# DeepGraphLearning/RNNLogic

Hardware: NVIDIA B200
Metric: rule_grounded_train_queries_per_sec (higher is better)
Workload: dtype u32/f32

## Files before the change

### rnnlogic_b200/csrc/rl_kernels.cu

```cuda
#include "rl_device.cuh"
#include <stdlib.h>

static thread_local char g_err[512] = "";
static long long g_launches = 0;

int rl_fail(int code, const char *what, cudaError_t e)
{
    if (e != cudaSuccess) snprintf(g_err, sizeof(g_err), "%s: %s", what, cudaGetErrorString(e));
    else snprintf(g_err, sizeof(g_err), "%s", what);
    return code;
}
void rl_count_launch() { ++g_launches; }
static int fail(int code, const char *what, cudaError_t e = cudaSuccess) { return rl_fail(code, what, e); }

__global__ void k_prepare_slots(rl_graph g, int S, const int32_t *__restrict__ slot_head,
                                const int32_t *__restrict__ q_off, const int64_t *__restrict__ all_h,
                                const int64_t *__restrict__ all_t, const int64_t *__restrict__ etr, int remove_query_edges,
                                int32_t *lane_h, int32_t *lane_t, int32_t *lane_eh, int32_t *lane_et)
{
    int i = blockIdx.x * blockDim.x + threadIdx.x;
    if (i >= S * RL_LANES) return;
    int s = i >> 5, lane = i & 31;
    int qi = q_off[s] + lane;
    bool valid = qi < q_off[s + 1];
    int64_t hv = valid ? all_h[qi] : -1, tv = (valid && all_t) ? all_t[qi] : -1;
    if (hv < 0 || hv >= g.num_entities) hv = -1;
    if (tv < 0 || tv >= g.num_entities) tv = -1;
    lane_h[i] = (int32_t)hv;
    lane_t[i] = (int32_t)tv;
    int eh = -1, et = -1;
    const int rel = slot_head[s];
    if (valid && etr) {
        int64_t k = etr[qi];
        int64_t n = g.ord_ptr[rel + 1] - g.ord_ptr[rel];
        if (k >= 0 && k < n) {
            eh = g.ord_h[g.ord_ptr[rel] + k];
            et = g.ord_t[g.ord_ptr[rel] + k];
        }
    } else if (valid && remove_query_edges && hv >= 0 && tv >= 0) {
        const int row = rank_row(g, rel, (int)tv);
        if (row >= 0) {
            const long long grow = g.dst_ptr[rel] + row;
            for (long long k = g.row_start[grow]; k < g.row_start[grow + 1]; ++k)
                if (g.edge_src[k] == (int)hv) { eh = (int)hv; et = (int)tv; break; }
        }
    }
    lane_eh[i] = eh;
    lane_et[i] = et;
}

__device__ __forceinline__ int srank_row(const rl_graph &g, int rel, int e)
{
    const uint2 w = __ldg(reinterpret_cast<const uint2 *>(g.srank_tab) + (size_t)rel * g.rank_words + (e >> 5));
    const uint32_t bit = 1u << (e & 31);
    return (w.x & bit) ? (int)(w.y + __popc(w.x & (bit - 1))) : -1;
}

__device__ __forceinline__ void mark_out_edges(const rl_graph &g, int rho, int ent, uint32_t *cm)
{
    const int sr = srank_row(g, rho, ent);
    if (sr < 0) return;
    const int fb = g.fsrc_ptr[rho] + sr;
    const int k1 = g.frow_start[fb + 1];
    for (int k = g.frow_start[fb]; k < k1; ++k) {
        const int dr = __ldg(g.fedge_dstrow + k);
        atomicOr(cm + (dr >> 5), 1u << (dr & 31));
    }
}

template <bool ROOT>
__global__ void __launch_bounds__(WARPS_PER_BLOCK * 32)
k_symbolic(rl_graph g, rl_rules r, rl_slots s, int depth, rl_frontier fr, int dense_num, int dense_den, int force_dense)
{
    const int lane = threadIdx.x & 31, warp = threadIdx.x >> 5;
    const int slot = blockIdx.y;
    const int q = s.slot_head[slot];
    const int32_t *ip = r.lvl_sym_ptr + (size_t)q * (r.max_len + 1);
    const int item = ip[depth - 1] + blockIdx.x * WARPS_PER_BLOCK + warp;
    if (item >= ip[depth]) return;
    const int v = r.sym_node[item], w0 = r.sym_w0[item];
    const int4 ra = __ldg(reinterpret_cast<const int4 *>(r.node_rec) + 2 * (size_t)v);
    const int4 rb4 = __ldg(reinterpret_cast<const int4 *>(r.node_rec) + 2 * (size_t)v + 1);
    const int rho = ra.x;
    const int D = rb4.x;
    const int nw = (D + 31) >> 5;
    if (nw == 0) return;
    const int hc0 = r.lvl_ptr[(size_t)q * (r.max_len + 1)];
    uint32_t *mbase = fr.row_mask + (size_t)s.mask_off[slot];
    uint32_t *cm = mbase + (rb4.y - hc0);
    const int nzb = s.nz_off[slot] - r.head_node_ptr[q];
    bool dense = force_dense != 0;
    const uint32_t *pm = nullptr;
    int rho_p = -1, Dp = 0;
    if (!ROOT) {
        const int p = ra.y;
        const int cntp = fr.node_cnt[nzb + p];
        if (!dense && cntp == 0) return;
        rho_p = ra.z;
        Dp = g.dst_ptr[rho_p + 1] - g.dst_ptr[rho_p];
        if ((long long)cntp * dense_den > (long long)Dp * dense_num) dense = true;
        pm = mbase + (rb4.z - hc0);
    }
    if (dense) {
        if (w0 == 0)
            for (int w = lane; w < nw; w += 32)
                cm[w] = (w == nw - 1 && (D & 31)) ? ((1u << (D & 31)) - 1u) : 0xffffffffu;
        return;
    }
    if (ROOT) {
        const int h = s.lane_h[slot * RL_LANES + lane];
        if (h >= 0) mark_out_edges(g, rho, h, cm);
    } else {
        const int nwp = (Dp + 31) >> 5;
        const int pb = g.dst_ptr[rho_p];
        const int wi = w0 + lane;
        uint32_t word = wi < nwp ? pm[wi] : 0u;
        const int mine = __popc(word);
        int P = mine;
#pragma unroll
        for (int o = 1; o < 32; o <<= 1) {
            const int t = __shfl_up_sync(FULL, P, o);
            if (lane >= o) P += t;
        }
        const int T = __shfl_sync(FULL, P, 31);
        const int first = P - mine;
        for (int base = 0; base < T; base += 32) {
            const int k = min(base + lane, T - 1);
            int src_lane = 0;
#pragma unroll
            for (int step = 16; step > 0; step >>= 1)
                if (__shfl_sync(FULL, P, src_lane + step - 1) <= k) src_lane += step;
            const uint32_t wsel = __shfl_sync(FULL, word, src_lane);
            const int nth = k - __shfl_sync(FULL, first, src_lane);
            if (base + lane < T) {
                const int bit = __fns(wsel, 0, nth + 1);
                mark_out_edges(g, rho, __ldg(g.row_dst + pb + (w0 + src_lane) * 32 + bit), cm);
            }
        }
    }
}

#define EDGE_GROUP 8
#ifndef NUM_WARPS
#define NUM_WARPS 4
#endif
template <typename CT, bool ROOT, bool PRUNE>
__device__ __forceinline__ uint32_t numeric_rows(const rl_graph &g, const rl_rules &r, const rl_slots &s, const rl_frontier &fr,
                                                 int slot, int q, int hc0, const uint32_t *mbase, int v, int myrow,
                                                 int h, int lane_eh, int lane_et, bool &ovf)
{
    const int lane = threadIdx.x & 31;
    const int4 ra = __ldg(reinterpret_cast<const int4 *>(r.node_rec) + 2 * (size_t)v);
    const int4 rb4 = __ldg(reinterpret_cast<const int4 *>(r.node_rec) + 2 * (size_t)v + 1);
    const int rho = ra.x, prel = ra.z, nterm = rb4.w;
    const size_t abase = (size_t)s.arena_off[slot];
    CT *arena = reinterpret_cast<CT *>(fr.arena);
    const CT *__restrict__ X = nullptr;
    const uint32_t *__restrict__ pm = nullptr;
    if (!ROOT) {
        X = arena + (abase + (size_t)r.node_prow_off[v]) * RL_LANES;
        pm = mbase + (rb4.z - hc0);
    }
    CT *__restrict__ Y = arena + (abase + (size_t)r.node_row_off[v]) * RL_LANES;
    const bool active = myrow >= 0;
    const int grow = ra.w + max(myrow, 0);
    const int my_dst = active ? g.row_dst[grow] : -1;
    const bool masked = (rho == q);
    const int eh = masked ? lane_eh : -1;
    const int et = masked ? lane_et : -1;

    int cur = -1;
    unsigned long long acc = 0;
    uint32_t nzrows = 0;
    uint32_t my_lanes = 0;
    auto flush = [&](int j) {
        if (masked) {
            const int d = __shfl_sync(FULL, my_dst, j);
            if (eh >= 0 && et == d) {
                unsigned long long sub;
                if (ROOT) sub = (eh == h) ? 1ull : 0ull;
                else {
                    int pr = rank_row(g, prel, eh);
                    if (pr >= 0 && !((pm[pr >> 5] >> (pr & 31)) & 1u)) pr = -1;
                    sub = pr >= 0 ? (unsigned long long)X[(size_t)pr * RL_LANES + lane] : 0ull;
                }
                acc -= sub;
            }
        }
        if (sizeof(CT) == 4 && (acc >> 32)) ovf = true;
        const uint32_t nzl = __ballot_sync(FULL, acc != 0);
        if (!PRUNE || nzl) {
            Y[(size_t)__shfl_sync(FULL, myrow, j) * RL_LANES + lane] = (CT)acc;
            nzrows |= 1u << j;
            if (lane == j) my_lanes = nzl;
        }
        acc = 0;
    };

    constexpr bool SEARCH = ROOT && PRUNE;
    if (SEARCH) {
        int fs = 0, fe = 0;
        if (h >= 0) {
            const int sr = srank_row(g, rho, h);
            if (sr >= 0) {
                const int fb = g.fsrc_ptr[rho] + sr;
                fs = g.frow_start[fb];
                fe = g.frow_start[fb + 1];
            }
        }
        for (uint32_t act = __ballot_sync(FULL, active); act; act &= act - 1) {
            const int j = __ffs(act) - 1;
            const int rj = __shfl_sync(FULL, myrow, j);
            int lo = fs, hi = fe;
            while (lo < hi) {
                const int mid = (lo + hi) >> 1;
                if (__ldg(g.fedge_dstrow + mid) < rj) lo = mid + 1; else hi = mid;
            }
            int cnt = 0;
            while (lo + cnt < fe && __ldg(g.fedge_dstrow + lo + cnt) == rj) ++cnt;
            acc = (unsigned long long)cnt;
            flush(j);
        }
    } else {
    const int32_t *__restrict__ rs = ROOT ? g.row_start + grow : r.pair_ptr + (r.node_pair_off[v] + max(myrow, 0));
    const int my_rs = active ? rs[0] : 0;
    const int my_re = active ? rs[1] : 0;
    const int deg = my_re - my_rs;
    int P = deg;
#pragma unroll
    for (int o = 1; o < 32; o <<= 1) {
        const int t = __shfl_up_sync(FULL, P, o);
        if (lane >= o) P += t;
    }
    const int T = __shfl_sync(FULL, P, 31);
    const int my_first = P - deg;
    for (int base = 0; base < T; base += 32) {
        const int n = min(32, T - base);
        const int k = min(base + lane, T - 1);
        int row = 0;
#pragma unroll
        for (int step = 16; step > 0; step >>= 1)
            if (__shfl_sync(FULL, P, row + step - 1) <= k) row += step;
        const int e = __shfl_sync(FULL, my_rs, row) + (k - __shfl_sync(FULL, my_first, row));
        const int src = lane < n ? __ldg((ROOT ? g.edge_src : r.pair_ent) + e) : -1;
        int pr = -1;
        if (!ROOT && src >= 0 && ((pm[src >> 5] >> (src & 31)) & 1u)) pr = src;
        uint32_t todo = ROOT ? (n == 32 ? FULL : ((1u << n) - 1u)) : __ballot_sync(FULL, pr >= 0);
        while (todo) {
            CT vals[EDGE_GROUP];
            int rws[EDGE_GROUP];
#pragma unroll
            for (int u = 0; u < EDGE_GROUP; ++u) {
                const int kk = todo ? __ffs(todo) - 1 : -1;
                todo &= todo - 1;
                rws[u] = kk >= 0 ? __shfl_sync(FULL, row, kk) : -1;
                if (ROOT) {
                    const int sv = __shfl_sync(FULL, src, kk & 31);
                    vals[u] = (CT)((kk >= 0) && (sv == h));
                } else {
                    const int p = __shfl_sync(FULL, pr, kk & 31);
                    vals[u] = kk >= 0 ? X[(size_t)p * RL_LANES + lane] : (CT)0;
                }
            }
#pragma unroll
            for (int u = 0; u < EDGE_GROUP; ++u) {
                if (rws[u] >= 0) {
                    if (rws[u] != cur) {
                        if (cur >= 0) flush(cur);
                        cur = rws[u];
                    }
                    acc += (unsigned long long)vals[u];
                }
            }
        }
    }
    if (cur >= 0) flush(cur);
    }
    if (nterm > 0 && nzrows) {
        const bool mine = (nzrows >> lane) & 1u;
        if (fr.items) {
            const int term0 = __ldg(r.node_term_ptr + v);
            int base = 0;
            if (lane == 0) base = atomicAdd(fr.item_cnt + slot, __popc(nzrows));
            base = __shfl_sync(FULL, base, 0);
            if (mine) {
                const long long pos = fr.item_off[slot] + base + __popc(nzrows & ((1u << lane) - 1u));
                reinterpret_cast<int4 *>(fr.items)[pos] = make_int4((int)(r.node_row_off[v] + myrow), term0, my_dst, nterm);
                if (fr.item_mask) fr.item_mask[pos] = my_lanes;
                if (fr.bucket_cnt) atomicAdd(fr.bucket_cnt + (size_t)slot * RL_BUCKET_STRIDE(g.rank_words) + my_dst, 1);
                else if (fr.nzmask && my_lanes) atomicOr(fr.nzmask + (size_t)slot * g.num_entities + my_dst, my_lanes);
            }
        }
    }
    return nzrows;
}

template <typename CT, bool ROOT, bool PRUNE>
__global__ void __launch_bounds__(NUM_WARPS * 32, 48 / NUM_WARPS)
k_numeric(rl_graph g, rl_rules r, rl_slots s, int depth, rl_frontier fr, int cpw)
{
    const int lane = threadIdx.x & 31, warp = threadIdx.x >> 5;
    const int slot = blockIdx.y;
    const int q = s.slot_head[slot];
    const int32_t *lp = r.lvl_ptr + (size_t)q * (r.max_len + 1);
    const int c_end = lp[depth];
    const int c0 = lp[depth - 1] + (blockIdx.x * NUM_WARPS + warp) * cpw;
    if (c0 >= c_end) return;
    const int hc0 = lp[0];
    uint32_t *mbase = fr.row_mask + (size_t)s.mask_off[slot];
    const int nzb = s.nz_off[slot] - r.head_node_ptr[q];
    const int my_chunk = c0 + lane;
    const bool mine = lane < cpw && my_chunk < c_end;
    const uint32_t my_m = mine ? mbase[my_chunk - hc0] : 0u;
    uint32_t todo = __ballot_sync(FULL, my_m != 0u);
    if (todo == 0u) return;
    const int my_node = my_m ? r.chunk_node[my_chunk] : -1;
    const int my_row0 = my_m ? r.chunk_row0[my_chunk] : 0;
    const int h = s.lane_h[slot * RL_LANES + lane];
    const int leh = s.lane_eh[slot * RL_LANES + lane];
    const int let_ = s.lane_et[slot * RL_LANES + lane];
    bool ovf = false;
    int rows_done = 0;
    while (todo) {
        const int v = __shfl_sync(FULL, my_node, __ffs(todo) - 1);
        const uint32_t seg = __ballot_sync(FULL, my_m != 0u && my_node == v);
        todo &= ~seg;
        const int cnt = ((seg >> lane) & 1u) ? __popc(my_m) : 0;
        int P = cnt;
#pragma unroll
        for (int o = 1; o < 32; o <<= 1) {
            const int t = __shfl_up_sync(FULL, P, o);
            if (lane >= o) P += t;
        }
        const int V = __shfl_sync(FULL, P, 31);
        const int first = P - cnt;
        for (int g0 = 0; g0 < V; g0 += 32) {
            const bool have = g0 + lane < V;
            const int k = min(g0 + lane, V - 1);
            int sl = 0;
#pragma unroll
            for (int step = 16; step > 0; step >>= 1)
                if (__shfl_sync(FULL, P, sl + step - 1) <= k) sl += step;
            const uint32_t wsel = __shfl_sync(FULL, my_m, sl);
            const int nth = k - __shfl_sync(FULL, first, sl);
            const int r0 = __shfl_sync(FULL, my_row0, sl);
            const int bit = __fns(wsel, 0, nth + 1);
            const int myrow = have ? r0 + bit : -1;
            const uint32_t nz = numeric_rows<CT, ROOT, PRUNE>(g, r, s, fr, slot, q, hc0, mbase, v, myrow, h, leh, let_, ovf);
            if (have && !((nz >> lane) & 1u)) atomicAnd(mbase + (c0 + sl - hc0), ~(1u << bit));
            if (lane == 0 && nz) atomicAdd(fr.node_cnt + nzb + v, __popc(nz));
            rows_done += __popc(nz);
        }
    }
    if (lane == 0 && rows_done && depth < 8) atomicAdd(fr.overflow + 1 + depth, rows_done);
    if (__any_sync(FULL, ovf) && lane == 0) fr.overflow[0] = 1;
}

template <bool FILL>
__global__ void __launch_bounds__(128)
k_pair_table(rl_graph g, const int32_t *__restrict__ pair_prel, const int32_t *__restrict__ pair_rel,
             const int64_t *__restrict__ pair_base, const int32_t *__restrict__ ptr, int32_t *__restrict__ out)
{
    const int p = blockIdx.x;
    const int rp = pair_prel[p], rr = pair_rel[p];
    const long long base = pair_base[p];
    const int row0 = g.dst_ptr[rr], D = g.dst_ptr[rr + 1] - row0;
    for (int d = threadIdx.x; d < D; d += blockDim.x) {
        int n = 0;
        const int pos = FILL ? ptr[base + d] : 0;
        const int k1 = g.row_start[row0 + d + 1];
        for (int k = g.row_start[row0 + d]; k < k1; ++k) {
            const int pr = rank_row(g, rp, __ldg(g.edge_src + k));
            if (pr >= 0) {
                if (FILL) out[pos + n] = pr;
                ++n;
            }
        }
        if (!FILL) out[base + d] = n;
    }
    if (!FILL && threadIdx.x == 0) out[base + D] = 0;
}

__global__ void __launch_bounds__(WARPS_PER_BLOCK * 32)
k_propagate_dense(rl_graph g, int rel, int B, const int64_t *__restrict__ x, const int64_t *__restrict__ etr,
                  int64_t *__restrict__ out)
{
    const int lane = threadIdx.x & 31, warp = threadIdx.x >> 5;
    const int e = blockIdx.x * WARPS_PER_BLOCK + warp;
    if (e >= g.num_entities) return;
    const int row = rank_row(g, rel, e);
    const long long o0 = g.ord_ptr[rel], n_ord = g.ord_ptr[rel + 1] - o0;
    for (int b = lane; b < B; b += 32) {
        unsigned long long acc = 0;
        if (row >= 0) {
            const long long grow = g.dst_ptr[rel] + row;
            for (int k = g.row_start[grow]; k < g.row_start[grow + 1]; ++k)
                acc += (unsigned long long)x[(size_t)g.edge_src[k] * B + b];
            if (etr) {
                const long long k = etr[b];
                if (k >= 0 && k < n_ord && g.ord_t[o0 + k] == e) acc -= (unsigned long long)x[(size_t)g.ord_h[o0 + k] * B + b];
            }
        }
        out[(size_t)e * B + b] = (int64_t)acc;
    }
}

template <typename CT>
__global__ void k_node_dense(rl_graph g, rl_rules r, rl_slots s, int slot, int node, rl_frontier fr,
                             int64_t *__restrict__ out)
{
    __shared__ long long tile[32][33];
    const int lane = threadIdx.x & 31, w = threadIdx.x >> 5;
    const int N = g.num_entities;
    const int e = blockIdx.x * 32 + w;
    long long c = 0;
    if (e < N) {
        if (node < 0) c = (s.lane_h[slot * RL_LANES + lane] == e);
        else {
            const int q = s.slot_head[slot];
            const int hc0 = r.lvl_ptr[(size_t)q * (r.max_len + 1)];
            const uint32_t *mbase = fr.row_mask + (size_t)s.mask_off[slot];
            const int row = rank_row(g, r.node_rel[node], e);
            if (row >= 0 && row_valid(r.node_chunk0, mbase, hc0, node, row))
                c = (long long)reinterpret_cast<const CT *>(fr.arena)[((size_t)s.arena_off[slot] + r.node_row_off[node] + row) * RL_LANES + lane];
        }
    }
    tile[w][lane] = c;
    __syncthreads();
    const int eo = blockIdx.x * 32 + lane;
    if (eo < N) out[(size_t)w * N + eo] = tile[lane][w];
}

__global__ void __launch_bounds__(512)
k_items_scan(int W, rl_frontier fr)
{
    __shared__ int wsum[16];
    const int slot = blockIdx.x, tid = threadIdx.x, lane = tid & 31, warp = tid >> 5;
    int4 *cnt4 = reinterpret_cast<int4 *>(fr.bucket_cnt + (size_t)slot * RL_BUCKET_STRIDE(W));
    int4 *off4 = reinterpret_cast<int4 *>(fr.bucket_off + (size_t)slot * RL_BUCKET_STRIDE(W));
    int carry = 0;
    for (int w0 = 0; w0 < W; w0 += 512) {
        const int w = w0 + tid;
        int4 c[8];
        int sum = 0;
        if (w < W) {
#pragma unroll
            for (int k = 0; k < 8; ++k) {
                c[k] = cnt4[(size_t)w * 8 + k];
                sum += (c[k].x + c[k].y) + (c[k].z + c[k].w);
            }
        }
        int incl = sum;
#pragma unroll
        for (int o = 1; o < 32; o <<= 1) {
            const int v = __shfl_up_sync(FULL, incl, o);
            if (lane >= o) incl += v;
        }
        if (lane == 31) wsum[warp] = incl;
        __syncthreads();
        int wbase = 0, total = 0;
#pragma unroll
        for (int k = 0; k < 16; ++k) {
            const int v = wsum[k];
            if (k < warp) wbase += v;
            total += v;
        }
        int run = carry + wbase + incl - sum;
        if (w < W) {
#pragma unroll
            for (int k = 0; k < 8; ++k) {
                int4 o;
                o.x = run; run += c[k].x;
                o.y = run; run += c[k].y;
                o.z = run; run += c[k].z;
                o.w = run; run += c[k].w;
                off4[(size_t)w * 8 + k] = o;
                cnt4[(size_t)w * 8 + k] = make_int4(0, 0, 0, 0);
            }
        }
        carry += total;
        __syncthreads();
    }
    if (tid == 0) fr.bucket_off[(size_t)slot * RL_BUCKET_STRIDE(W) + (size_t)W * 32] = carry;
}

#define SCATTER_BLOCKS 16
__global__ void __launch_bounds__(256)
k_items_scatter(int N, int W, rl_frontier fr)
{
    const int slot = blockIdx.y;
    int *cnt = fr.bucket_cnt + (size_t)slot * RL_BUCKET_STRIDE(W);
    const int *off = fr.bucket_off + (size_t)slot * RL_BUCKET_STRIDE(W);
    const int n = fr.item_cnt[slot];
    const int4 *in = reinterpret_cast<const int4 *>(fr.items) + fr.item_off[slot];
    int4 *out = reinterpret_cast<int4 *>(fr.items_sorted) + fr.item_off[slot];
    const uint32_t *min_ = fr.item_mask ? fr.item_mask + fr.item_off[slot] : nullptr;
    uint32_t *mout = fr.item_mask_sorted ? fr.item_mask_sorted + fr.item_off[slot] : nullptr;
    uint32_t *nz = fr.nzmask ? fr.nzmask + (size_t)slot * N : nullptr;
    for (int i = blockIdx.x * 256 + threadIdx.x; i < n; i += SCATTER_BLOCKS * 256) {
        const int4 it = in[i];
        const int pos = off[it.z] + atomicAdd(cnt + it.z, 1);
        out[pos] = it;
        if (min_ && mout) {
            const uint32_t m = min_[i];
            mout[pos] = m;
            if (nz && m) atomicOr(nz + it.z, m);
        }
    }
}

static int launch_items_sort(const rl_graph *g, const rl_slots *s, const rl_frontier *fr, cudaStream_t st)
{
    k_items_scan<<<s->num_slots, 512, 0, st>>>(g->rank_words, *fr);
    CHECK_LAUNCH("k_items_scan");
    k_items_scatter<<<dim3(SCATTER_BLOCKS, s->num_slots), 256, 0, st>>>(g->num_entities, g->rank_words, *fr);
    CHECK_LAUNCH("k_items_scatter");
    return RL_OK;
}

template <typename CT>
__global__ void __launch_bounds__(SCORE_WARPS_MAX * 32, SCORE_MIN_BLOCKS)       
k_predictor_scores(rl_graph g, rl_rules r, rl_slots s, rl_frontier fr, const float *__restrict__ w,
                   const float *__restrict__ bias, int fill_neg_inf, float *__restrict__ Z,
// ... 831 lines not shown
```

Before: 4.914 million.

## Replace per-row binary searches with warp-wide merge of sorted edge list

In the root search path, each active row used to run its own binary search over the lane's sorted destination-row edge list. The new code does one binary search to the smallest row, then walks the edge list once and binary-searches the warp's sorted row keys with shuffles to mark hits. Rows with several edges fall back to the old per-row counting search. This replaces up to 32 binary searches with a single linear merge, but the merge length grows with how many edges fall in the row range, and it assumes the active rows are sorted and packed into the low lanes.

Result: faster. 5.117 million (median of 6 runs) (+4.1%).

```diff
diff --git a/rnnlogic_b200/csrc/rl_kernels.cu b/rnnlogic_b200/csrc/rl_kernels.cu
--- a/rnnlogic_b200/csrc/rl_kernels.cu
+++ b/rnnlogic_b200/csrc/rl_kernels.cu
@@ -1,4 +1,5 @@
 #include "rl_device.cuh"
+#include <limits.h>
 #include <stdlib.h>
 
 static thread_local char g_err[512] = "";
@@ -199,26 +200,55 @@
 
     constexpr bool SEARCH = ROOT && PRUNE;
     if (SEARCH) {
-        int fs = 0, fe = 0;
-        if (h >= 0) {
-            const int sr = srank_row(g, rho, h);
+        auto own_edges = [&](int &fs, int &fe) {
+            fs = fe = 0;
+            const int sr = h >= 0 ? srank_row(g, rho, h) : -1;
             if (sr >= 0) {
                 const int fb = g.fsrc_ptr[rho] + sr;
                 fs = g.frow_start[fb];
                 fe = g.frow_start[fb + 1];
             }
-        }
-        for (uint32_t act = __ballot_sync(FULL, active); act; act &= act - 1) {
-            const int j = __ffs(act) - 1;
+        };
+        int lo, fe;
+        own_edges(lo, fe);
+        const uint32_t act = __ballot_sync(FULL, active);
+        const int key = active ? myrow : INT_MAX;
+        const int r_lo = __shfl_sync(FULL, myrow, 0), r_hi = __shfl_sync(FULL, myrow, __popc(act) - 1);
+        for (int hi = fe; lo < hi;) {
+            const int mid = (lo + hi) >> 1;
+            if (__ldg(g.fedge_dstrow + mid) < r_lo) lo = mid + 1; else hi = mid;
+        }
+        uint32_t hit = 0;
+        bool multi = false;
+        int d = lo < fe ? __ldg(g.fedge_dstrow + lo) : INT_MAX;
+        while (__any_sync(FULL, d <= r_hi)) {
+            int j = 0;
+#pragma unroll
+            for (int step = 16; step > 0; step >>= 1)
+                if (__shfl_sync(FULL, key, j + step - 1) < d) j += step;
+            const bool match = __shfl_sync(FULL, key, j & 31) == d && j < 32 && d <= r_hi;
+            if (match) {
+                multi |= (hit >> j) & 1u;
+                hit |= 1u << j;
+            }
+            if (d <= r_hi) d = ++lo < fe ? __ldg(g.fedge_dstrow + lo) : INT_MAX;
+        }
+        for (uint32_t todo = act; todo; todo &= todo - 1) {
+            const int j = __ffs(todo) - 1;
             const int rj = __shfl_sync(FULL, myrow, j);
-            int lo = fs, hi = fe;
-            while (lo < hi) {
-                const int mid = (lo + hi) >> 1;
-                if (__ldg(g.fedge_dstrow + mid) < rj) lo = mid + 1; else hi = mid;
-            }
-            int cnt = 0;
-            while (lo + cnt < fe && __ldg(g.fedge_dstrow + lo + cnt) == rj) ++cnt;
-            acc = (unsigned long long)cnt;
+            acc = (hit >> j) & 1u;
+            if (multi && acc) {
+                int a, b;
+                own_edges(a, b);
+                const int end = b;
+                while (a < b) {
+                    const int mid = (a + b) >> 1;
+                    if (__ldg(g.fedge_dstrow + mid) < rj) a = mid + 1; else b = mid;
+                }
+                int cnt = 0;
+                while (a + cnt < end && __ldg(g.fedge_dstrow + a + cnt) == rj) ++cnt;
+                acc = (unsigned long long)cnt;
+            }
             flush(j);
         }
     } else {
```
